# MrGreyPanda/NEM-MCMC-optimization

Hardware: AMD Instinct MI355X
Metric: order-score evals/sec (64 S-genes x 2000 effects); HBM GB/s fraction (higher is better)
Workload: dtype int8 fixed point 2^-38/ln2 + fp64 LSE

## Files before the change

nem-mcmc-optimization_amd/csrc/nemo_factored_i8.hip:

```cpp
#include "nemo_internal.h"

#include <math.h>

#include <string.h>

#include <algorithm>
#include <cmath>
#include <vector>

#ifndef NEMO_I8_ABLATE
#define NEMO_I8_ABLATE 0
#endif
#ifndef NEMO_I8L_RINIT
#define NEMO_I8L_RINIT 1
#endif
#ifndef NEMO_I8_WAVES_PER_SIMD
#define NEMO_I8_WAVES_PER_SIMD 2
#endif

namespace nemo {

namespace {

using i32x4 = __attribute__((ext_vector_type(4))) int;

constexpr double kPadG8 = -1.0e6;
constexpr int kARow = 6;
template <int ROWC>
__device__ __forceinline__ int a_byte(int i, int j) {
  if constexpr (ROWC == 4) return i * 64 + (((j >> 4) + 2 * ((i >> 2) & 3)) & 3) * 16 + (j & 15);
  else return i * (16 * ROWC) + j;
}

__device__ __forceinline__ double wsum(double v) {
#pragma unroll
  for (int o = 32; o >= 1; o >>= 1) v += __shfl_xor(v, o, kWave);
  return v;
// ... 129 lines not shown
  A8[1 * SL + off] = (int8_t)(((hb >> 12) & 63) - 32);
  A8[2 * SL + off] = (int8_t)(((hb >> 6) & 63) - 32);
  A8[3 * SL + off] = (int8_t)((hb & 63) - 32);
  A8[4 * SL + off] = (int8_t)(lb >> 18);
  A8[5 * SL + off] = (int8_t)(((lb >> 12) & 63) - 32);
  A8[6 * SL + off] = (int8_t)(((lb >> 6) & 63) - 32);
  A8[7 * SL + off] = (int8_t)((lb & 63) - 32);
}

constexpr double kL2Scale = 1512775.3951951857;

template <int SPAD, int ROWC>
__device__ __forceinline__ void i8l_digits(int8_t* A8, int i, int j, double d) {
  const double hd = rint(d * kL2Scale);
  const int h = (int)hd;
  const int l = (int)rint(fma(d, kL2Scale, -hd) * 262144.0);
  const int off = a_byte<ROWC>(i, j);
  const int hb = h + 32 * (1 + 64 + 4096), lb = l + 32 * (1 + 64);
  constexpr int SL = SPAD * 16 * ROWC;
  A8[0 * SL + off] = (int8_t)(hb >> 18);
  A8[1 * SL + off] = (int8_t)(((hb >> 12) & 63) - 32);
  A8[2 * SL + off] = (int8_t)(((hb >> 6) & 63) - 32);
  A8[3 * SL + off] = (int8_t)((hb & 63) - 32);
  A8[4 * SL + off] = (int8_t)(lb >> 12);
  A8[5 * SL + off] = (int8_t)(((lb >> 6) & 63) - 32);
  A8[6 * SL + off] = (int8_t)((lb & 63) - 32);
}

__device__ __forceinline__ double dswap32(double a, double b, double& out_b) {
  const uint64_t x = __builtin_bit_cast(uint64_t, a), y = __builtin_bit_cast(uint64_t, b);
  auto lo = __builtin_amdgcn_permlane32_swap((uint32_t)x, (uint32_t)y, false, false);
  auto hi = __builtin_amdgcn_permlane32_swap((uint32_t)(x >> 32), (uint32_t)(y >> 32), false, false);
  out_b = __builtin_bit_cast(double, ((uint64_t)hi[1] << 32) | lo[1]);
  return __builtin_bit_cast(double, ((uint64_t)hi[0] << 32) | lo[0]);
}
__device__ __forceinline__ double dswap16(double a, double b, double& out_b) {
  const uint64_t x = __builtin_bit_cast(uint64_t, a), y = __builtin_bit_cast(uint64_t, b);
  auto lo = __builtin_amdgcn_permlane16_swap((uint32_t)x, (uint32_t)y, false, false);
  auto hi = __builtin_amdgcn_permlane16_swap((uint32_t)(x >> 32), (uint32_t)(y >> 32), false, false);
  out_b = __builtin_bit_cast(double, ((uint64_t)hi[1] << 32) | lo[1]);
  return __builtin_bit_cast(double, ((uint64_t)hi[0] << 32) | lo[0]);
}

template <int SPAD, int WAVES, int KB, int ROWC, bool L2 = false>
__device__ __forceinline__ void i8o_prep_passes(EvalLds e, int k0, int w, int lane, int S, int cap,
                                                int cexp, const double* __restrict__ w01b,
                                                const double* __restrict__ elo_s,
// ... 324 lines not shown

constexpr double kL2C0 = 1.0000000000000377;
constexpr double kL2C1 = 2.521654728528023e-12;
constexpr double kL2C2 = 3.179908378901339e-24;

__device__ __forceinline__ uint64_t exp2_fx_load(uint32_t t0) {
#if NEMO_I8_ABLATE & 64
  const uint32_t addr = 0u;
#else
  const uint32_t addr = (t0 >> 6) & 0x3ff8u;
#endif
  return *(const __attribute__((address_space(3))) uint64_t*)(size_t)addr;
}
__device__ __forceinline__ double exp2_fx_series(uint32_t t0, int t1) {
  uint32_t rr;
  asm("v_lshl_add_u32 %0, %1, 18, %2" : "=v"(rr) : "v"(t0 & 511u), "v"((uint32_t)t1));
  const double r = (double)(int)rr;
  return fma(r, fma(r, kL2C2, kL2C1), kL2C0);
}
__device__ __forceinline__ double exp2_fx_series_r(int rr) {
  const double r = (double)rr;
  return fma(r, fma(r, kL2C2, kL2C1), kL2C0);
}
__device__ __forceinline__ double exp2_fx_apply(uint32_t t0, uint64_t ev, double p, double acc) {
  const uint32_t hi = (t0 & ~511u) ^ (uint32_t)(ev >> 32);
  return fma(__builtin_bit_cast(double, ((uint64_t)hi << 32) | (uint32_t)ev), p, acc);
}

template <int NR, int WAVES, bool DIAG>
__global__ __launch_bounds__(WAVES * kWave, NEMO_I8O_WAVES_PER_SIMD) void score_i8o_kernel(
    int S, int E, int ntiles, int nsets, int split, int cap, int cexp, double padg,
    const int32_t* __restrict__ pos, const double* __restrict__ w01,
    const double* __restrict__ e_lo, const double* __restrict__ e_hi,
    const uint8_t* __restrict__ B8, const double* __restrict__ Uoff,
    const int8_t* __restrict__ udig, const double* __restrict__ u0,
    const double* __restrict__ nullsum, const void* __restrict__ tabs, double sA, double sB,
    double* __restrict__ partial, double* __restrict__ ll_out, int remap) {
  constexpr int SPAD = NR * 16;
  constexpr int NP = 4;
  constexpr int NSL = 2 * NP;
  extern __shared__ __attribute__((aligned(16))) double lds8[];
  uint2* etab_o = (uint2*)lds8;
  double2* ltab = (double2*)(etab_o + kExpTabN);
  double* elo_s = (double*)(ltab + 128);
  double* ehi_s = elo_s + SPAD;
  EvalLds ev;
// ... 147 lines not shown
  }
}

template <int NR, int WAVES, bool DIAG>
hipError_t launch_i8o_t(Ctx& c, int batch, int cap, const int32_t* d_pos, const double* d_w01,
                        double* d_ll, hipStream_t st, int* nparts, bool* finalized) {
  constexpr int SPAD = NR * 16;
  const int ntiles = (c.E + 15) / 16;
  const int nsets = (ntiles + 7) / 8;
  const int slots = 256 * (NEMO_I8O_WAVES_PER_SIMD * 4 / WAVES);
  int split = (slots + batch - 1) / batch;
  split = split < 1 ? 1 : (split > nsets ? nsets : split);
  const size_t lds = kExpTabN * 8 + 128 * 16 + 3 * SPAD * 8 + 3 * SPAD * 4 + (size_t)8 * SPAD * 64;
  const double sA = ldexp(1.0, c.i8_cexp - 24), sB = ldexp(1.0, c.i8_cexp - 48);
  score_i8o_kernel<NR, WAVES, DIAG><<<dim3(batch * split), WAVES * kWave, lds, st>>>(
      c.S, c.E, ntiles, nsets, split, cap, c.i8_cexp, c.i8o_padg, d_pos, d_w01, c.d_elo, c.d_ehi,
      c.d_B8, c.d_Uoff, c.d_udig, c.d_u0, c.d_nullsum, c.d_i8o_tabs, sA, sB, fpartial(c), d_ll,
      c.xcd_remap);
  *nparts = nsets;
  *finalized = split == 1;
  return hipGetLastError();
}

template <int NR, int WAVES, class Hook>
__device__ __forceinline__ int i8l_walk2(const i32x4* __restrict__ Al0, const i32x4* __restrict__ Gi,
                                        const i32x4* __restrict__ Bt, const i32x4* __restrict__ Bt64,
                                        int set, int s_end, int ntiles, int E, int col, int lane,
                                        uint32_t a_lane, const double* __restrict__ nullsum,
                                        double* __restrict__ partial, size_t b, int nsets,
                                        const double2* __restrict__ ltab, Hook hook) {
  constexpr int SPAD = NR * 16;
  const int rg = lane >> 4;
  int it = 0;
  if (set < s_end) {
    double lprod = 1.0;
    int lexp = 0;
    int t = 8 * set;
    auto tend = [&](int st) { return min(ntiles, 8 * st + 8); };
    int t2 = t + 1 < tend(set) ? t + 1 : t;
    const __amdgpu_buffer_rsrc_t brs =
        __builtin_amdgcn_make_buffer_rsrc((void*)Bt, (short)0, 2 * ntiles * kWave * 16, 0x00020000);
    const uint32_t bln = (uint32_t)lane * 16u;
    auto bload = [&](int tile, int x64) {
      return __builtin_bit_cast(i32x4, __builtin_amdgcn_raw_buffer_load_b128(
                                           brs, bln, (x64 * ntiles + tile) * kWave * 16, 0));
    };
    i32x4 bca = bload(t, 0), bca64 = bload(t, 1);
    i32x4 bcb = bload(t2, 0), bcb64 = bload(t2, 1);
    for (;;) {
      uint32_t ao = a_lane;
      asm volatile("" : "+v"(ao));
      const i32x4* Al = Al0 + ao;
      const bool two = t2 != t;
      int tn = t + 2, setn = set;
      if (tn >= tend(set)) {
        setn = set + WAVES;
        tn = 8 * setn;
      }
      const bool more = setn < s_end;
      const int tla = __builtin_amdgcn_readfirstlane(more ? tn : t);
      const int tlb = __builtin_amdgcn_readfirstlane(more ? (tn + 1 < tend(setn) ? tn + 1 : tn) : t);
      const i32x4 b1a = bca, b64a = bca64, b1b = bcb, b64b = bcb64;
      bca = bload(tla, 0);
      bca64 = bload(tla, 1);
      bcb = bload(tlb, 0);
      bcb64 = bload(tlb, 1);
      double la0 = 0.0, la1 = 0.0, lb0 = 0.0, lb1 = 0.0;
#pragma unroll
      for (int r = 0; r < NR; ++r) {
        const i32x4 c0 = Gi[(16 * r) / 4 + rg];
        const i32x4 c1 = Gi[(SPAD + 16 * r) / 4 + rg];
        auto A = [&](int sl) { return Al[(sl * SPAD + 16 * r) * 4]; };
        i32x4 h0a, h0b, h1a, h1b, l0a, l0b, l1a, l1b;
        {
          const i32x4 a = A(0);
          h0a = __builtin_amdgcn_mfma_i32_16x16x64_i8(a, b64a, i32x4{0, 0, 0, 0}, 0, 0, 0);
          h0b = __builtin_amdgcn_mfma_i32_16x16x64_i8(a, b64b, i32x4{0, 0, 0, 0}, 0, 0, 0);
        }
        {
          const i32x4 a = A(1);
          h0a = __builtin_amdgcn_mfma_i32_16x16x64_i8(a, b1a, h0a, 0, 0, 0);
          h0b = __builtin_amdgcn_mfma_i32_16x16x64_i8(a, b1b, h0b, 0, 0, 0);
        }
        {
          const i32x4 a = A(2);
          h1a = __builtin_amdgcn_mfma_i32_16x16x64_i8(a, b64a, c0, 0, 0, 0);
          h1b = __builtin_amdgcn_mfma_i32_16x16x64_i8(a, b64b, c0, 0, 0, 0);
        }
        {
          const i32x4 a = A(3);
          h1a = __builtin_amdgcn_mfma_i32_16x16x64_i8(a, b1a, h1a, 0, 0, 0);
          h1b = __builtin_amdgcn_mfma_i32_16x16x64_i8(a, b1b, h1b, 0, 0, 0);
        }
#if NEMO_I8L_RINIT
        {
          const i32x4 a = A(5);
          l1a = __builtin_amdgcn_mfma_i32_16x16x64_i8(a, b64a, c1, 0, 0, 0);
          l1b = __builtin_amdgcn_mfma_i32_16x16x64_i8(a, b64b, c1, 0, 0, 0);
        }
        {
          const i32x4 a = A(6);
          l1a = __builtin_amdgcn_mfma_i32_16x16x64_i8(a, b1a, l1a, 0, 0, 0);
          l1b = __builtin_amdgcn_mfma_i32_16x16x64_i8(a, b1b, l1b, 0, 0, 0);
        }
        uint32_t t0a[4], t0b[4];
        uint64_t eva[4], evb[4];
        i32x4 ma, mb;
#pragma unroll
        for (int g = 0; g < 4; ++g) {
          t0a[g] = ((uint32_t)h0a[g] << 12) + (uint32_t)h1a[g];
          eva[g] = exp2_fx_load(t0a[g]);
          ma[g] = (int)((t0a[g] & 511u) << 6);
        }
#pragma unroll
        for (int g = 0; g < 4; ++g) {
          t0b[g] = ((uint32_t)h0b[g] << 12) + (uint32_t)h1b[g];
          evb[g] = exp2_fx_load(t0b[g]);
          mb[g] = (int)((t0b[g] & 511u) << 6);
        }
        {
          const i32x4 a = A(4);
          l0a = __builtin_amdgcn_mfma_i32_16x16x64_i8(a, b1a, ma, 0, 0, 0);
          l0b = __builtin_amdgcn_mfma_i32_16x16x64_i8(a, b1b, mb, 0, 0, 0);
        }
        auto epi = [&](const uint32_t (&t0)[4], const uint64_t (&evv)[4], const i32x4 l0, const i32x4 l1,
                       double& ls0, double& ls1) {
          double pr[4];
#pragma unroll
          for (int g = 0; g < 4; ++g) pr[g] = exp2_fx_series_r((int)(((uint32_t)l0[g] << 12) + (uint32_t)l1[g]));
#pragma unroll
          for (int g = 0; g < 4; ++g) {
            if (g & 1) ls1 = exp2_fx_apply(t0[g], evv[g], pr[g], ls1);
            else ls0 = exp2_fx_apply(t0[g], evv[g], pr[g], ls0);
          }
        };
        epi(t0a, eva, l0a, l1a, la0, la1);
        epi(t0b, evb, l0b, l1b, lb0, lb1);
#else
        {
          const i32x4 a = A(4);
          l0a = __builtin_amdgcn_mfma_i32_16x16x64_i8(a, b1a, i32x4{0, 0, 0, 0}, 0, 0, 0);
          l0b = __builtin_amdgcn_mfma_i32_16x16x64_i8(a, b1b, i32x4{0, 0, 0, 0}, 0, 0, 0);
        }
        {
          const i32x4 a = A(5);
          l1a = __builtin_amdgcn_mfma_i32_16x16x64_i8(a, b64a, c1, 0, 0, 0);
          l1b = __builtin_amdgcn_mfma_i32_16x16x64_i8(a, b64b, c1, 0, 0, 0);
        }
        {
          const i32x4 a = A(6);
          l1a = __builtin_amdgcn_mfma_i32_16x16x64_i8(a, b1a, l1a, 0, 0, 0);
          l1b = __builtin_amdgcn_mfma_i32_16x16x64_i8(a, b1b, l1b, 0, 0, 0);
        }
        auto epi = [&](const i32x4 h0, const i32x4 h1, const i32x4 l0, const i32x4 l1, double& ls0,
                       double& ls1) {
          uint32_t t0[4];
          uint64_t evv[4];
          double pr[4];
#pragma unroll
          for (int g = 0; g < 4; ++g) {
            t0[g] = ((uint32_t)h0[g] << 12) + (uint32_t)h1[g];
            evv[g] = exp2_fx_load(t0[g]);
          }
#pragma unroll
          for (int g = 0; g < 4; ++g)
            pr[g] = exp2_fx_series(t0[g], (int)(((uint32_t)l0[g] << 12) + (uint32_t)l1[g]));
#pragma unroll
          for (int g = 0; g < 4; ++g) {
            if (g & 1) ls1 = exp2_fx_apply(t0[g], evv[g], pr[g], ls1);
            else ls0 = exp2_fx_apply(t0[g], evv[g], pr[g], ls0);
          }
        };
        epi(h0a, h1a, l0a, l1a, la0, la1);
        epi(h0b, h1b, l0b, l1b, lb0, lb1);
#endif
      }
      const double l = rowsum_pair(la0 + la1, lb0 + lb1) + 1.0;
      const bool tb = (lane & 16) != 0;
      const bool ok = (((tb ? t2 : t) * 16 + col) < E) & (two | !tb);
      lprod *= ok ? l : 1.0;
      lexp += __builtin_amdgcn_frexp_exp(lprod);
      lprod = __builtin_amdgcn_frexp_mant(lprod);
      if (setn != set) {
        double v = log_fast(lprod, ltab) + (double)lexp * 0.69314718055994530942;
        v = rowsum16(v);
        v += __shfl_down(v, 16, kWave);
        if (lane == 0) partial[(size_t)b * nsets + set] = nullsum[set] + v;
        lprod = 1.0;
        lexp = 0;
      }
      hook(it++);
      if (!more) break;
      t = tn;
      t2 = tlb;
      set = setn;
    }
  }
  return it;
}

template <int NR, int WAVES, int OCC, int TT = 1, int MODE = 0>
__global__ __launch_bounds__(WAVES * kWave, OCC) void score_i8l_kernel(
    int S, int E, int ntiles, int nsets, int split, int cap, double padg,
    const int32_t* __restrict__ pos, const double* __restrict__ w01,
    const double* __restrict__ e_lo, const double* __restrict__ e_hi,
    const uint8_t* __restrict__ B8, const int8_t* __restrict__ udig, const double* __restrict__ u0,
    const double* __restrict__ nullsum, const void* __restrict__ tabs,
    double* __restrict__ partial, double* __restrict__ ll_out, int remap,
    int4* __restrict__ img = nullptr) {
  constexpr int SPAD = NR * 16;
  constexpr int NSL = 7;
  extern __shared__ __attribute__((aligned(16))) double lds8[];
  uint2* etab_o = (uint2*)lds8;
  double2* ltab = (double2*)(etab_o + kExpTabN);
  double* elo_s = (double*)(ltab + 128);
  double* ehi_s = elo_s + SPAD;
  EvalLds ev;
  ev.G = ehi_s + SPAD;
// ... 17 lines not shown
    const int4* src = (const int4*)tabs;
    int4* dst = (int4*)lds8;
    for (int k = tid + (MODE == 1 ? kExpTabN * 8 / 16 : 0); k < (kExpTabN * 8 + 128 * 16) / 16;
         k += blockDim.x)
      dst[k] = src[k];
    if constexpr (MODE != 2)
      for (int i = tid; i < SPAD; i += blockDim.x) {
        elo_s[i] = i < S ? e_lo[i] : 1.0;
        ehi_s[i] = i < S ? e_hi[i] : 1.0;
      }
  }
  if constexpr (MODE == 2) {
    const int4* src = img + (size_t)b * kImg4;
    int4* dst = (int4*)gi;
    for (int k = tid; k < kImg4; k += blockDim.x) dst[k] = src[k];
    __syncthreads();
  } else {
  i8_init_eval<SPAD, NSL, 4>(ev, pos + (size_t)b * S, S, tid, blockDim.x, padg);
  __syncthreads();
  {
    int8_t* A8 = (int8_t*)ev.A;
    for (int k = tid; k < S * NSL; k += blockDim.x) {
      const int i = k / NSL, sl = k - i * NSL;
      A8[sl * SPAD * 64 + a_byte<4>(i, i)] = udig[i * 8 + sl];
    }
  }
  {
    constexpr int KB = 4;
    const int npass = i8_npass(S, cap);
    const int my = npass > w ? (npass - w + WAVES - 1) / WAVES : 0;
    for (int k0 = 0; k0 < my; k0 += KB)
      i8o_prep_passes<SPAD, WAVES, KB, 4, true>(ev, k0, w, lane, S, cap, 0, w01 + (size_t)b * S * S,
                                                elo_s, ehi_s, ltab);
  }
  __syncthreads();
  for (int i = tid; i < SPAD; i += blockDim.x) {
    const double g = i < S ? ev.G[i] + u0[i] : ev.G[i];
    const double g0 = rint(g * kL2Scale);
    gi[i] = (int)g0 + (1023 << 20);
    gi[SPAD + i] = (int)rint(fma(g, kL2Scale, -g0) * 262144.0);
  }
  __syncthreads();
  if constexpr (MODE == 1) {
    const int4* src = (const int4*)gi;
    int4* dst = img + (size_t)b * kImg4;
    for (int k = tid; k < kImg4; k += blockDim.x) dst[k] = src[k];
    return;
// ... 42 lines not shown
  #endif
  #if NEMO_I8_ABLATE & 2
          const i32x4 h0 = A(0) + A(1) + b64, h1 = A(2) + A(3) + c0, l0 = A(4) + b1,
                      l1 = A(5) + A(6) + c1;
  #else
          i32x4 h0 = __builtin_amdgcn_mfma_i32_16x16x64_i8(A(0), b64, i32x4{0, 0, 0, 0}, 0, 0, 0);
          h0 = __builtin_amdgcn_mfma_i32_16x16x64_i8(A(1), b1, h0, 0, 0, 0);
          i32x4 h1 = __builtin_amdgcn_mfma_i32_16x16x64_i8(A(2), b64, c0, 0, 0, 0);
          h1 = __builtin_amdgcn_mfma_i32_16x16x64_i8(A(3), b1, h1, 0, 0, 0);
          const i32x4 l0 = __builtin_amdgcn_mfma_i32_16x16x64_i8(A(4), b1, i32x4{0, 0, 0, 0}, 0, 0, 0);
          i32x4 l1 = __builtin_amdgcn_mfma_i32_16x16x64_i8(A(5), b64, c1, 0, 0, 0);
          l1 = __builtin_amdgcn_mfma_i32_16x16x64_i8(A(6), b1, l1, 0, 0, 0);
  #endif
          uint32_t t0[4];
          uint64_t ev[4];
          double pr[4];
  #pragma unroll
          for (int g = 0; g < 4; ++g) {
            t0[g] = ((uint32_t)h0[g] << 12) + (uint32_t)h1[g];
            ev[g] = exp2_fx_load(t0[g]);
          }
  #pragma unroll
          for (int g = 0; g < 4; ++g)
            pr[g] = exp2_fx_series(t0[g], (int)(((uint32_t)l0[g] << 12) + (uint32_t)l1[g]));
  #pragma unroll
          for (int g = 0; g < 4; ++g) {
            if (g & 1) ls1 = exp2_fx_apply(t0[g], ev[g], pr[g], ls1);
            else ls0 = exp2_fx_apply(t0[g], ev[g], pr[g], ls0);
          }
        }
        double l = rowsum4(ls0 + ls1) + 1.0;
        lprod *= t * 16 + col < E ? l : 1.0;
        lexp += __builtin_amdgcn_frexp_exp(lprod);
        lprod = __builtin_amdgcn_frexp_mant(lprod);
        if (setn != set) {
          double v = log_fast(lprod, ltab) + (double)lexp * 0.69314718055994530942;
          v = rowsum16(v);
          if (lane == 0) partial[(size_t)b * nsets + set] = nullsum[set] + v;
          lprod = 1.0;
          lexp = 0;
        }
        if (!more) break;
        t = tn;
        set = setn;
      }
    }
  } else {
    i8l_walk2<NR, WAVES>(ev.A, Gi, Bt, Bt64, set, s_end, ntiles, E, col, lane, a_lane, nullsum, partial, b,
                         nsets, ltab, [](int) {});
  }
  if (split == 1) {
    __syncthreads();
    if (w == 0) {
      const double v = sum_partials(partial + (size_t)b * nsets, nsets, lane);
      if (lane == 0) ll_out[b] = v;
    }
  }
}

template <int NR>
__global__ __launch_bounds__(8 * kWave, NEMO_I8O_WAVES_PER_SIMD) void score_i8s_kernel(
    int S, int E, int ntiles, int nsets, int split, int cap, double padg,
    const int32_t* __restrict__ pos, const double* __restrict__ w01,
    const double* __restrict__ e_lo, const double* __restrict__ e_hi,
    const uint8_t* __restrict__ B8, const int8_t* __restrict__ udig, const double* __restrict__ u0,
    const double* __restrict__ nullsum, const void* __restrict__ tabs,
    double* __restrict__ partial, double* __restrict__ ll_out, int remap) {
  constexpr int WAVES = 8;
  constexpr int SPAD = NR * 16;
  constexpr int NSL = 7;
  constexpr int NG = WAVES / NR;
// ... 16 lines not shown
  const int s_begin = part * spb;
  const int s_end = min(nsets, s_begin + spb);
  const int tid = threadIdx.x;
  const int lane = tid & (kWave - 1);
  const int w = __builtin_amdgcn_readfirstlane(tid / kWave);
  const int rb = w % NR, grp = w / NR;
  const int col = lane & 15, rg = lane >> 4;

  {
    const int4* src = (const int4*)tabs;
    int4* dst = (int4*)lds8;
    for (int k = tid; k < (kExpTabN * 8 + 128 * 16) / 16; k += blockDim.x) dst[k] = src[k];
    for (int i = tid; i < SPAD; i += blockDim.x) {
      elo_s[i] = i < S ? e_lo[i] : 1.0;
      ehi_s[i] = i < S ? e_hi[i] : 1.0;
    }
  }
  i8_init_eval<SPAD, NSL, 4>(ev, pos + (size_t)b * S, S, tid, blockDim.x, padg);
  __syncthreads();
  {
    int8_t* A8 = (int8_t*)ev.A;
    for (int k = tid; k < S * NSL; k += blockDim.x) {
      const int i = k / NSL, sl = k - i * NSL;
      A8[sl * SPAD * 64 + a_byte<4>(i, i)] = udig[i * 8 + sl];
    }
  }
  {
    constexpr int KB = 4;
    const int npass = i8_npass(S, cap);
    const int my = npass > w ? (npass - w + WAVES - 1) / WAVES : 0;
    for (int k0 = 0; k0 < my; k0 += KB)
      i8o_prep_passes<SPAD, WAVES, KB, 4, true>(ev, k0, w, lane, S, cap, 0, w01 + (size_t)b * S * S,
                                                elo_s, ehi_s, ltab);
  }
  __syncthreads();
  for (int i = tid; i < SPAD; i += blockDim.x) {
    const double g = i < S ? ev.G[i] + u0[i] : ev.G[i];
    const double g0 = rint(g * kL2Scale);
    gi[i] = (int)g0 + (1023 << 20);
    gi[SPAD + i] = (int)rint(fma(g, kL2Scale, -g0) * 262144.0);
  }
  __syncthreads();
  i32x4 af[NSL];
  {
    const i32x4* Al = ev.A + (uint32_t)(col * 4 + ((rg + 2 * (col >> 2)) & 3));
#pragma unroll
    for (int sl = 0; sl < NSL; ++sl) af[sl] = Al[(sl * SPAD + 16 * rb) * 4];
// ... 17 lines not shown
      const int t_end = min(ntiles, 8 * set + 8);
      for (int t = 8 * set; t < t_end; ++t) {
        const int tn = t + 1 < t_end ? t + 1 : 8 * (set + NG);
        const i32x4 b1 = bc;
        const i32x4 b64 = b1 << 6;
        bc = Bt[(size_t)min(tn, ntiles - 1) * kWave + lane];
        const i32x4 h0 = __builtin_amdgcn_mfma_i32_16x16x64_i8(
            af[1], b1, __builtin_amdgcn_mfma_i32_16x16x64_i8(af[0], b64, i32x4{0, 0, 0, 0}, 0, 0, 0), 0, 0, 0);
        const i32x4 h1 = __builtin_amdgcn_mfma_i32_16x16x64_i8(
            af[3], b1, __builtin_amdgcn_mfma_i32_16x16x64_i8(af[2], b64, c0, 0, 0, 0), 0, 0, 0);
        const i32x4 l0 = __builtin_amdgcn_mfma_i32_16x16x64_i8(af[4], b1, i32x4{0, 0, 0, 0}, 0, 0, 0);
        const i32x4 l1 = __builtin_amdgcn_mfma_i32_16x16x64_i8(
            af[6], b1, __builtin_amdgcn_mfma_i32_16x16x64_i8(af[5], b64, c1, 0, 0, 0), 0, 0, 0);
        uint32_t t0[4];
        uint64_t evt[4];
        double pr[4];
#pragma unroll
        for (int g = 0; g < 4; ++g) {
          t0[g] = ((uint32_t)h0[g] << 12) + (uint32_t)h1[g];
          evt[g] = exp2_fx_load(t0[g]);
        }
#pragma unroll
        for (int g = 0; g < 4; ++g)
          pr[g] = exp2_fx_series(t0[g], (int)(((uint32_t)l0[g] << 12) + (uint32_t)l1[g]));
        double ls0 = 0.0, ls1 = 0.0;
#pragma unroll
        for (int g = 0; g < 4; ++g) {
          if (g & 1) ls1 = exp2_fx_apply(t0[g], evt[g], pr[g], ls1);
          else ls0 = exp2_fx_apply(t0[g], evt[g], pr[g], ls0);
        }
        const double v = rowsum4(ls0 + ls1);
        if (lane < 16) cs[((t - 8 * set) * NR + rb) * 16 + col] = v;
      }
    }
    __syncthreads();
    if (set < s_end && rb == k % NR) {
      double lp = 1.0;
      int le = 0;
#pragma unroll
      for (int h = 0; h < 2; ++h) {
        const int tt = (lane >> 4) + 4 * h;
        const int t = 8 * set + tt;
        double l = 1.0;
#pragma unroll
        for (int q = 0; q < NR; ++q) l += cs[(tt * NR + q) * 16 + col];
        lp *= t < ntiles && t * 16 + col < E ? l : 1.0;
        le += __builtin_amdgcn_frexp_exp(lp);
// ... 45 lines not shown
  const int lane = tid & (kWave - 1);
  const int w = __builtin_amdgcn_readfirstlane(tid / kWave);
  const int col = lane & 15, rg = lane >> 4;
  const int nb = gridDim.x;
  const int b0 = blockIdx.x;
  if (b0 >= batch) return;

  auto set_perm = [&](int k, int e) {
    int* perm = evb(k).perm;
    for (int j = tid; j < S; j += blockDim.x) {
      int pj = pos[(size_t)e * S + j];
      pj = pj < 0 ? 0 : (pj >= S ? S - 1 : pj);
      perm[pj] = j;
    }
  };
  auto zero_a = [&](int k) {
    i32x4* A = evb(k).A;
    for (int q = tid; q < NSL * SPAD * 4; q += blockDim.x) A[q] = i32x4{0, 0, 0, 0};
  };
  auto diag = [&](int k) {
    int8_t* A8 = (int8_t*)evb(k).A;
    for (int q = tid; q < S * NSL; q += blockDim.x) {
      const int i = q / NSL, sl = q - i * NSL;
      A8[sl * SPAD * 64 + a_byte<4>(i, i)] = udig[i * 8 + sl];
    }
  };
  auto prep = [&](int k, int e) {
    constexpr int KB = 4;
    const int npass = i8_npass(S, cap);
    const int my = npass > w ? (npass - w + WAVES - 1) / WAVES : 0;
    for (int k0 = 0; k0 < my; k0 += KB)
      i8o_prep_passes<SPAD, WAVES, KB, 4, true>(evb(k), k0, w, lane, S, cap, 0, w01 + (size_t)e * S * S,
                                                elo_s, ehi_s, ltab);
  };
  auto finalize_g = [&](int k) {
    const EvalLds ev = evb(k);
    int* gi = gib(k);
    for (int i = tid; i < SPAD; i += blockDim.x) {
      const double g = i < S ? ev.G[i] + u0[i] : ev.G[i];
      const double g0 = rint(g * kL2Scale);
      gi[i] = (int)g0 + (1023 << 20);
      gi[SPAD + i] = (int)rint(fma(g, kL2Scale, -g0) * 262144.0);
    }
  };

  {
    const int4* src = (const int4*)tabs;
// ... 6 lines not shown
  }
  for (int k = 0; k < 2; ++k) {
    for (int i = tid; i < SPAD; i += blockDim.x) evb(k).G[i] = i < S ? 0.0 : padg;
    zero_a(k);
  }
  set_perm(0, b0);
  if (b0 + nb < batch) set_perm(1, b0 + nb);
  __syncthreads();
  diag(0);
  diag(1);
  __syncthreads();
  prep(0, b0);
  __syncthreads();
  finalize_g(0);
  __syncthreads();

  const i32x4* Bt = (const i32x4*)B8;
  const i32x4* Bt64 = Bt + (size_t)ntiles * kWave;
  const uint32_t a_lane = (uint32_t)(col * 4 + ((rg + 2 * (col >> 2)) & 3));
  int k = 0;
  for (int e = b0; e < batch; e += nb, k ^= 1) {
    const int en = e + nb;
    bool pending = en < batch;
    i8l_walk2<NR, WAVES>(evb(k).A, (const i32x4*)gib(k), Bt, Bt64, w, nsets, ntiles, E, col, lane, a_lane,
                         nullsum, partial, (size_t)e, nsets, ltab, [&](int it) {
                           if (pending && it == 0) {
                             prep(k ^ 1, en);
                             pending = false;
                           }
                         });
    if (pending) prep(k ^ 1, en);
    __syncthreads();
    if (w == 0) {
      const double v = sum_partials(partial + (size_t)e * nsets, nsets, lane);
      if (lane == 0) ll_out[e] = v;
    }
    if (en < batch) finalize_g(k ^ 1);
    const bool again = en + nb < batch;
    if (again) {
      zero_a(k);
      set_perm(k, en + nb);
    }
    __syncthreads();
    if (again) diag(k);
  }
}

// ... 64 lines not shown
  } else {
    score_i8l_kernel<NR, WAVES, OCC, TT><<<dim3(batch * split), WAVES * kWave, lds, st>>>(
        c.S, c.E, ntiles, nsets, split, cap, c.i8o_padg, d_pos, d_w01, c.d_elo, c.d_ehi, c.d_B8,
        c.d_udig2, c.d_u0, c.d_nullsum, c.d_i8o_tabs, fpartial(c), d_ll, c.xcd_remap);
  }
  *nparts = nsets;
  *finalized = split == 1;
  return hipGetLastError();
}

constexpr int kWideKH = 2;

__device__ __forceinline__ void i8w_digits(int8_t* A8, int i, int j, double d) {
  constexpr int SPAD = 128, SL = SPAD * 64;
  const double hd = rint(d * kL2Scale);
  const int h = (int)hd;
  const int l = (int)rint(fma(d, kL2Scale, -hd) * 262144.0);
  const int off = (j >> 6) * SL + a_byte<4>(i, j & 63);
  const int hb = h + 32 * (1 + 64 + 4096), lb = l + 32 * (1 + 64);
  A8[(0 * kWideKH) * SL + off] = (int8_t)(hb >> 18);
  A8[(1 * kWideKH) * SL + off] = (int8_t)(((hb >> 12) & 63) - 32);
  A8[(2 * kWideKH) * SL + off] = (int8_t)(((hb >> 6) & 63) - 32);
  A8[(3 * kWideKH) * SL + off] = (int8_t)((hb & 63) - 32);
  A8[(4 * kWideKH) * SL + off] = (int8_t)(lb >> 12);
  A8[(5 * kWideKH) * SL + off] = (int8_t)(((lb >> 6) & 63) - 32);
  A8[(6 * kWideKH) * SL + off] = (int8_t)((lb & 63) - 32);
}

template <int WAVES, int KB>
__device__ __forceinline__ void i8w_prep_passes(EvalLds e, int k0, int w, int lane, int S, int cap,
                                                const double* __restrict__ w01b,
                                                const double* __restrict__ elo_s,
                                                const double* __restrict__ ehi_s,
                                                const double2* __restrict__ ltab) {
  const bool packed = cap == 0 || cap >= S - 1;
  const int npass = packed ? (S + 1) / 2 : S;
  int8_t* A8 = (int8_t*)e.A;
  double ga[KB], gb[KB];
#pragma unroll
  for (int kk = 0; kk < KB; ++kk) {
    ga[kk] = 0.0;
    gb[kk] = 0.0;
    const int q = w + (k0 + kk) * WAVES;
#pragma unroll
    for (int hr = 0; hr < kWideKH; ++hr) {
      const int p = lane + 64 * hr;
      int qr = 0, pp = 0;
// ... 57 lines not shown
  ev.A = (i32x4*)(ev.perm + SPAD);

  const int b = xcd_index8((int)blockIdx.x, (int)gridDim.x, remap);
  const int tid = threadIdx.x;
  const int lane = tid & (kWave - 1);
  const int w = __builtin_amdgcn_readfirstlane(tid / kWave);
  const int col = lane & 15, rg = lane >> 4;

  {
    const int4* src = (const int4*)tabs;
    int4* dst = (int4*)lds8;
    for (int k = tid; k < (kExpTabN * 8 + 128 * 16) / 16; k += blockDim.x) dst[k] = src[k];
    for (int i = tid; i < SPAD; i += blockDim.x) {
      elo_s[i] = i < S ? e_lo[i] : 1.0;
      ehi_s[i] = i < S ? e_hi[i] : 1.0;
    }
  }
  i8_init_eval<SPAD, NSL * kWideKH, 4>(ev, pos + (size_t)b * S, S, tid, blockDim.x, padg);
  __syncthreads();
  {
    int8_t* A8 = (int8_t*)ev.A;
    for (int k = tid; k < S * NSL; k += blockDim.x) {
      const int i = k / NSL, sl = k - i * NSL;
      A8[(sl * kWideKH + (i >> 6)) * SPAD * 64 + a_byte<4>(i, i & 63)] = udig[i * 8 + sl];
    }
  }
  {
    constexpr int KB = 2;
    const int npass = i8_npass(S, cap);
    const int my = npass > w ? (npass - w + WAVES - 1) / WAVES : 0;
    for (int k0 = 0; k0 < my; k0 += KB)
      i8w_prep_passes<WAVES, KB>(ev, k0, w, lane, S, cap, w01 + (size_t)b * S * S, elo_s, ehi_s, ltab);
  }
  __syncthreads();
  for (int i = tid; i < SPAD; i += blockDim.x) {
    const double g = i < S ? ev.G[i] + u0[i] : ev.G[i];
    const double g0 = rint(g * kL2Scale);
    gi[i] = (int)g0 + (1023 << 20);
    gi[SPAD + i] = (int)rint(fma(g, kL2Scale, -g0) * 262144.0);
  }
  __syncthreads();

  const i32x4* Gi = (const i32x4*)gi;
  const uint32_t a_lane = (uint32_t)(col * 4 + ((rg + 2 * (col >> 2)) & 3));
  const __amdgpu_buffer_rsrc_t brs =
      __builtin_amdgcn_make_buffer_rsrc((void*)B8, (short)0, 2 * kWideKH * ntiles * kWave * 16, 0x00020000);
  const uint32_t bln = (uint32_t)lane * 16u;
  auto bload = [&](int tile, int x64, int h) {
    return __builtin_bit_cast(i32x4, __builtin_amdgcn_raw_buffer_load_b128(
                                         brs, bln, ((x64 * kWideKH + h) * ntiles + tile) * kWave * 16, 0));
  };
  if constexpr (TWO) {
    for (int set = w; set < nsets; set += WAVES) {
      const int ta = kWideSetT * set;
      const bool two = ta + 1 < ntiles;
      const int tb = two ? ta + 1 : ta;
      const i32x4 b1a[2] = {bload(ta, 0, 0), bload(ta, 0, 1)}, b64a[2] = {bload(ta, 1, 0), bload(ta, 1, 1)};
      const i32x4 b1b[2] = {bload(tb, 0, 0), bload(tb, 0, 1)}, b64b[2] = {bload(tb, 1, 0), bload(tb, 1, 1)};
      uint32_t ao = a_lane;
      asm volatile("" : "+v"(ao));
      const i32x4* Al = ev.A + ao;
      double la0 = 0.0, la1 = 0.0, lb0 = 0.0, lb1 = 0.0;
#pragma unroll 1
      for (int r = 0; r < NR; ++r) {
        const i32x4 c0 = Gi[(16 * r) / 4 + rg];
        const i32x4 c1 = Gi[(SPAD + 16 * r) / 4 + rg];
        auto A = [&](int sl, int h) { return Al[((sl * kWideKH + h) * SPAD + 16 * r) * 4]; };
        i32x4 h0a = i32x4{0, 0, 0, 0}, h0b = i32x4{0, 0, 0, 0}, h1a = c0, h1b = c0;
        i32x4 l0a = i32x4{0, 0, 0, 0}, l0b = i32x4{0, 0, 0, 0}, l1a = c1, l1b = c1;
#pragma unroll
        for (int h = 0; h < kWideKH; ++h) {
          {
            const i32x4 a = A(0, h);
            h0a = __builtin_amdgcn_mfma_i32_16x16x64_i8(a, b64a[h], h0a, 0, 0, 0);
            h0b = __builtin_amdgcn_mfma_i32_16x16x64_i8(a, b64b[h], h0b, 0, 0, 0);
          }
          {
            const i32x4 a = A(1, h);
            h0a = __builtin_amdgcn_mfma_i32_16x16x64_i8(a, b1a[h], h0a, 0, 0, 0);
            h0b = __builtin_amdgcn_mfma_i32_16x16x64_i8(a, b1b[h], h0b, 0, 0, 0);
          }
          {
            const i32x4 a = A(2, h);
            h1a = __builtin_amdgcn_mfma_i32_16x16x64_i8(a, b64a[h], h1a, 0, 0, 0);
            h1b = __builtin_amdgcn_mfma_i32_16x16x64_i8(a, b64b[h], h1b, 0, 0, 0);
          }
          {
            const i32x4 a = A(3, h);
            h1a = __builtin_amdgcn_mfma_i32_16x16x64_i8(a, b1a[h], h1a, 0, 0, 0);
            h1b = __builtin_amdgcn_mfma_i32_16x16x64_i8(a, b1b[h], h1b, 0, 0, 0);
          }
          {
            const i32x4 a = A(4, h);
            l0a = __builtin_amdgcn_mfma_i32_16x16x64_i8(a, b1a[h], l0a, 0, 0, 0);
            l0b = __builtin_amdgcn_mfma_i32_16x16x64_i8(a, b1b[h], l0b, 0, 0, 0);
          }
          {
            const i32x4 a = A(5, h);
            l1a = __builtin_amdgcn_mfma_i32_16x16x64_i8(a, b64a[h], l1a, 0, 0, 0);
            l1b = __builtin_amdgcn_mfma_i32_16x16x64_i8(a, b64b[h], l1b, 0, 0, 0);
          }
          {
            const i32x4 a = A(6, h);
            l1a = __builtin_amdgcn_mfma_i32_16x16x64_i8(a, b1a[h], l1a, 0, 0, 0);
            l1b = __builtin_amdgcn_mfma_i32_16x16x64_i8(a, b1b[h], l1b, 0, 0, 0);
          }
        }
        auto epi = [&](const i32x4 h0, const i32x4 h1, const i32x4 l0, const i32x4 l1, double& ls0,
                       double& ls1) {
          uint32_t t0[4];
          uint64_t evv[4];
          double pr[4];
#pragma unroll
          for (int g = 0; g < 4; ++g) {
            t0[g] = ((uint32_t)h0[g] << 12) + (uint32_t)h1[g];
            evv[g] = exp2_fx_load(t0[g]);
          }
#pragma unroll
          for (int g = 0; g < 4; ++g)
            pr[g] = exp2_fx_series(t0[g], (int)(((uint32_t)l0[g] << 12) + (uint32_t)l1[g]));
#pragma unroll
          for (int g = 0; g < 4; ++g) {
            if (g & 1) ls1 = exp2_fx_apply(t0[g], evv[g], pr[g], ls1);
            else ls0 = exp2_fx_apply(t0[g], evv[g], pr[g], ls0);
          }
        };
        epi(h0a, h1a, l0a, l1a, la0, la1);
        epi(h0b, h1b, l0b, l1b, lb0, lb1);
      }
      const double l = rowsum_pair(la0 + la1, lb0 + lb1) + 1.0;
      const bool tile_b = (lane & 16) != 0;
      const bool ok = (((tile_b ? tb : ta) * 16 + col) < E) & (two | !tile_b);
      const double lprod = ok ? l : 1.0;
      double v = log_fast(lprod, ltab);
      v = rowsum16(v);
      v += __shfl_down(v, 16, kWave);
      if (lane == 0) partial[(size_t)b * nsets + set] = nullsum[set] + v;
    }
  } else {
    for (int set = w; set < nsets; set += WAVES) {
      double lprod = 1.0;
      int lexp = 0;
      const int t_end = min(ntiles, kWideSetT * set + kWideSetT);
      for (int t = kWideSetT * set; t < t_end; ++t) {
        const i32x4 b1[2] = {bload(t, 0, 0), bload(t, 0, 1)};
        const i32x4 b64[2] = {bload(t, 1, 0), bload(t, 1, 1)};
        uint32_t ao = a_lane;
        asm volatile("" : "+v"(ao));
        const i32x4* Al = ev.A + ao;
        double ls0 = 0.0, ls1 = 0.0;
  #pragma unroll 2
// ... 5 lines not shown
          h0 = __builtin_amdgcn_mfma_i32_16x16x64_i8(A(0, 1), b64[1], h0, 0, 0, 0);
          h0 = __builtin_amdgcn_mfma_i32_16x16x64_i8(A(1, 0), b1[0], h0, 0, 0, 0);
          h0 = __builtin_amdgcn_mfma_i32_16x16x64_i8(A(1, 1), b1[1], h0, 0, 0, 0);
          i32x4 h1 = __builtin_amdgcn_mfma_i32_16x16x64_i8(A(2, 0), b64[0], c0, 0, 0, 0);
          h1 = __builtin_amdgcn_mfma_i32_16x16x64_i8(A(2, 1), b64[1], h1, 0, 0, 0);
          h1 = __builtin_amdgcn_mfma_i32_16x16x64_i8(A(3, 0), b1[0], h1, 0, 0, 0);
          h1 = __builtin_amdgcn_mfma_i32_16x16x64_i8(A(3, 1), b1[1], h1, 0, 0, 0);
          i32x4 l0 = __builtin_amdgcn_mfma_i32_16x16x64_i8(A(4, 0), b1[0], i32x4{0, 0, 0, 0}, 0, 0, 0);
          l0 = __builtin_amdgcn_mfma_i32_16x16x64_i8(A(4, 1), b1[1], l0, 0, 0, 0);
          i32x4 l1 = __builtin_amdgcn_mfma_i32_16x16x64_i8(A(5, 0), b64[0], c1, 0, 0, 0);
          l1 = __builtin_amdgcn_mfma_i32_16x16x64_i8(A(5, 1), b64[1], l1, 0, 0, 0);
          l1 = __builtin_amdgcn_mfma_i32_16x16x64_i8(A(6, 0), b1[0], l1, 0, 0, 0);
          l1 = __builtin_amdgcn_mfma_i32_16x16x64_i8(A(6, 1), b1[1], l1, 0, 0, 0);
          uint32_t t0[4];
          uint64_t evv[4];
          double pr[4];
  #pragma unroll
          for (int g = 0; g < 4; ++g) {
            t0[g] = ((uint32_t)h0[g] << 12) + (uint32_t)h1[g];
            evv[g] = exp2_fx_load(t0[g]);
          }
  #pragma unroll
          for (int g = 0; g < 4; ++g)
            pr[g] = exp2_fx_series(t0[g], (int)(((uint32_t)l0[g] << 12) + (uint32_t)l1[g]));
  #pragma unroll
          for (int g = 0; g < 4; ++g) {
            if (g & 1) ls1 = exp2_fx_apply(t0[g], evv[g], pr[g], ls1);
            else ls0 = exp2_fx_apply(t0[g], evv[g], pr[g], ls0);
          }
        }
        const double l = rowsum4(ls0 + ls1) + 1.0;
        lprod *= t * 16 + col < E ? l : 1.0;
        lexp += __builtin_amdgcn_frexp_exp(lprod);
        lprod = __builtin_amdgcn_frexp_mant(lprod);
      }
      double v = log_fast(lprod, ltab) + (double)lexp * 0.69314718055994530942;
      v = rowsum16(v);
      if (lane == 0) partial[(size_t)b * nsets + set] = nullsum[set] + v;
    }
  }
  __syncthreads();
  if (w == 0) {
    const double v = sum_partials(partial + (size_t)b * nsets, nsets, lane);
    if (lane == 0) ll_out[b] = v;
  }
}

// ... 264 lines not shown
```

Baseline: 14.27 million.

## Fold low-residual init into MFMA accumulator and ping-pong B prefetch registers

Doubles the stored slice-4 digit and shifts the l0 partial by 11 instead of 12. The (t0 & 511) residual is now seeded into the l0 MFMA accumulator through a 16-bit shift, so the series no longer has to add it separately. The wide kernel now runs its l0 MFMAs after the table lookup and uses the cheaper series_r path. The walk loop is also turned into a lambda that is unrolled twice, swapping two B register sets instead of copying them each iteration. All of this reorders MFMA and epilogue work to cut VALU operations and register moves, at the cost of touching the fixed-point digit encoding, which risks numeric range issues.

```diff
diff --git a/nem-mcmc-optimization_amd/csrc/nemo_factored_i8.hip b/nem-mcmc-optimization_amd/csrc/nemo_factored_i8.hip
--- a/nem-mcmc-optimization_amd/csrc/nemo_factored_i8.hip
+++ b/nem-mcmc-optimization_amd/csrc/nemo_factored_i8.hip
@@ -13,6 +13,12 @@
 #endif
 #ifndef NEMO_I8L_RINIT
 #define NEMO_I8L_RINIT 1
+#endif
+#ifndef NEMO_I8L_CINIT16
+#define NEMO_I8L_CINIT16 1
+#endif
+#ifndef NEMO_I8L_PINGPONG
+#define NEMO_I8L_PINGPONG 1
 #endif
 #ifndef NEMO_I8_WAVES_PER_SIMD
 #define NEMO_I8_WAVES_PER_SIMD 2
@@ -188,7 +194,7 @@
   A8[1 * SL + off] = (int8_t)(((hb >> 12) & 63) - 32);
   A8[2 * SL + off] = (int8_t)(((hb >> 6) & 63) - 32);
   A8[3 * SL + off] = (int8_t)((hb & 63) - 32);
-  A8[4 * SL + off] = (int8_t)(lb >> 12);
+  A8[4 * SL + off] = (int8_t)(2 * (lb >> 12));
   A8[5 * SL + off] = (int8_t)(((lb >> 6) & 63) - 32);
   A8[6 * SL + off] = (int8_t)((lb & 63) - 32);
 }
@@ -559,6 +565,15 @@
   const double r = (double)rr;
   return fma(r, fma(r, kL2C2, kL2C1), kL2C0);
 }
+__device__ __forceinline__ int i8l_cinit16(uint32_t t0) {
+#if NEMO_I8L_CINIT16
+  int r;
+  asm("v_lshlrev_b16 %0, 7, %1" : "=v"(r) : "v"(t0));
+  return r;
+#else
+  return (int)((t0 & 511u) << 7);
+#endif
+}
 __device__ __forceinline__ double exp2_fx_apply(uint32_t t0, uint64_t ev, double p, double acc) {
   const uint32_t hi = (t0 & ~511u) ^ (uint32_t)(ev >> 32);
   return fma(__builtin_bit_cast(double, ((uint64_t)hi << 32) | (uint32_t)ev), p, acc);
@@ -752,7 +767,7 @@
   return hipGetLastError();
 }
 
-template <int NR, int WAVES, class Hook>
+template <int NR, int WAVES, bool PP, class Hook>
 __device__ __forceinline__ int i8l_walk2(const i32x4* __restrict__ Al0, const i32x4* __restrict__ Gi,
                                         const i32x4* __restrict__ Bt, const i32x4* __restrict__ Bt64,
                                         int set, int s_end, int ntiles, int E, int col, int lane,
@@ -777,7 +792,8 @@
     };
     i32x4 bca = bload(t, 0), bca64 = bload(t, 1);
     i32x4 bcb = bload(t2, 0), bcb64 = bload(t2, 1);
-    for (;;) {
+    auto iter = [&](const i32x4 b1a, const i32x4 b64a, const i32x4 b1b, const i32x4 b64b, i32x4& na,
+                    i32x4& na64, i32x4& nb, i32x4& nb64) -> bool {
       uint32_t ao = a_lane;
       asm volatile("" : "+v"(ao));
       const i32x4* Al = Al0 + ao;
@@ -790,11 +806,10 @@
       const bool more = setn < s_end;
       const int tla = __builtin_amdgcn_readfirstlane(more ? tn : t);
       const int tlb = __builtin_amdgcn_readfirstlane(more ? (tn + 1 < tend(setn) ? tn + 1 : tn) : t);
-      const i32x4 b1a = bca, b64a = bca64, b1b = bcb, b64b = bcb64;
-      bca = bload(tla, 0);
-      bca64 = bload(tla, 1);
-      bcb = bload(tlb, 0);
-      bcb64 = bload(tlb, 1);
+      na = bload(tla, 0);
+      na64 = bload(tla, 1);
+      nb = bload(tlb, 0);
+      nb64 = bload(tlb, 1);
       double la0 = 0.0, la1 = 0.0, lb0 = 0.0, lb1 = 0.0;
 #pragma unroll
       for (int r = 0; r < NR; ++r) {
@@ -840,13 +855,13 @@
         for (int g = 0; g < 4; ++g) {
           t0a[g] = ((uint32_t)h0a[g] << 12) + (uint32_t)h1a[g];
           eva[g] = exp2_fx_load(t0a[g]);
-          ma[g] = (int)((t0a[g] & 511u) << 6);
+          ma[g] = i8l_cinit16(t0a[g]);
         }
 #pragma unroll
         for (int g = 0; g < 4; ++g) {
           t0b[g] = ((uint32_t)h0b[g] << 12) + (uint32_t)h1b[g];
           evb[g] = exp2_fx_load(t0b[g]);
-          mb[g] = (int)((t0b[g] & 511u) << 6);
+          mb[g] = i8l_cinit16(t0b[g]);
         }
         {
           const i32x4 a = A(4);
@@ -857,7 +872,7 @@
                        double& ls0, double& ls1) {
           double pr[4];
 #pragma unroll
-          for (int g = 0; g < 4; ++g) pr[g] = exp2_fx_series_r((int)(((uint32_t)l0[g] << 12) + (uint32_t)l1[g]));
+          for (int g = 0; g < 4; ++g) pr[g] = exp2_fx_series_r((int)(((uint32_t)l0[g] << 11) + (uint32_t)l1[g]));
 #pragma unroll
           for (int g = 0; g < 4; ++g) {
             if (g & 1) ls1 = exp2_fx_apply(t0[g], evv[g], pr[g], ls1);
@@ -894,7 +909,7 @@
           }
 #pragma unroll
           for (int g = 0; g < 4; ++g)
-            pr[g] = exp2_fx_series(t0[g], (int)(((uint32_t)l0[g] << 12) + (uint32_t)l1[g]));
+            pr[g] = exp2_fx_series(t0[g], (int)(((uint32_t)l0[g] << 11) + (uint32_t)l1[g]));
 #pragma unroll
           for (int g = 0; g < 4; ++g) {
             if (g & 1) ls1 = exp2_fx_apply(t0[g], evv[g], pr[g], ls1);
@@ -920,10 +935,28 @@
         lexp = 0;
       }
       hook(it++);
-      if (!more) break;
+      if (!more) return false;
       t = tn;
       t2 = tlb;
       set = setn;
+      return true;
+    };
+    if constexpr (PP) {
+      i32x4 bqa, bqa64, bqb, bqb64;
+      for (;;) {
+        if (!iter(bca, bca64, bcb, bcb64, bqa, bqa64, bqb, bqb64)) break;
+        if (!iter(bqa, bqa64, bqb, bqb64, bca, bca64, bcb, bcb64)) break;
+      }
+    } else {
+      for (;;) {
+        i32x4 na, na64, nb, nb64;
+        const bool more = iter(bca, bca64, bcb, bcb64, na, na64, nb, nb64);
+        bca = na;
+        bca64 = na64;
+        bcb = nb;
+        bcb64 = nb64;
+        if (!more) break;
+      }
     }
   }
   return it;
@@ -987,7 +1020,8 @@
     int8_t* A8 = (int8_t*)ev.A;
     for (int k = tid; k < S * NSL; k += blockDim.x) {
       const int i = k / NSL, sl = k - i * NSL;
-      A8[sl * SPAD * 64 + a_byte<4>(i, i)] = udig[i * 8 + sl];
+      const int8_t d = udig[i * 8 + sl];
+      A8[sl * SPAD * 64 + a_byte<4>(i, i)] = sl == 4 ? (int8_t)(2 * d) : d;
     }
   }
   {
@@ -1076,7 +1110,7 @@
           }
   #pragma unroll
           for (int g = 0; g < 4; ++g)
-            pr[g] = exp2_fx_series(t0[g], (int)(((uint32_t)l0[g] << 12) + (uint32_t)l1[g]));
+            pr[g] = exp2_fx_series(t0[g], (int)(((uint32_t)l0[g] << 11) + (uint32_t)l1[g]));
   #pragma unroll
           for (int g = 0; g < 4; ++g) {
             if (g & 1) ls1 = exp2_fx_apply(t0[g], ev[g], pr[g], ls1);
@@ -1100,7 +1134,7 @@
       }
     }
   } else {
-    i8l_walk2<NR, WAVES>(ev.A, Gi, Bt, Bt64, set, s_end, ntiles, E, col, lane, a_lane, nullsum, partial, b,
+    i8l_walk2<NR, WAVES, NEMO_I8L_PINGPONG != 0>(ev.A, Gi, Bt, Bt64, set, s_end, ntiles, E, col, lane, a_lane, nullsum, partial, b,
                          nsets, ltab, [](int) {});
   }
   if (split == 1) {
@@ -1163,7 +1197,8 @@
     int8_t* A8 = (int8_t*)ev.A;
     for (int k = tid; k < S * NSL; k += blockDim.x) {
       const int i = k / NSL, sl = k - i * NSL;
-      A8[sl * SPAD * 64 + a_byte<4>(i, i)] = udig[i * 8 + sl];
+      const int8_t d = udig[i * 8 + sl];
+      A8[sl * SPAD * 64 + a_byte<4>(i, i)] = sl == 4 ? (int8_t)(2 * d) : d;
     }
   }
   {
@@ -1227,7 +1262,7 @@
         }
 #pragma unroll
         for (int g = 0; g < 4; ++g)
-          pr[g] = exp2_fx_series(t0[g], (int)(((uint32_t)l0[g] << 12) + (uint32_t)l1[g]));
+          pr[g] = exp2_fx_series(t0[g], (int)(((uint32_t)l0[g] << 11) + (uint32_t)l1[g]));
         double ls0 = 0.0, ls1 = 0.0;
 #pragma unroll
         for (int g = 0; g < 4; ++g) {
@@ -1319,7 +1354,8 @@
     int8_t* A8 = (int8_t*)evb(k).A;
     for (int q = tid; q < S * NSL; q += blockDim.x) {
       const int i = q / NSL, sl = q - i * NSL;
-      A8[sl * SPAD * 64 + a_byte<4>(i, i)] = udig[i * 8 + sl];
+      const int8_t d = udig[i * 8 + sl];
+      A8[sl * SPAD * 64 + a_byte<4>(i, i)] = sl == 4 ? (int8_t)(2 * d) : d;
     }
   };
   auto prep = [&](int k, int e) {
@@ -1372,7 +1408,7 @@
   for (int e = b0; e < batch; e += nb, k ^= 1) {
     const int en = e + nb;
     bool pending = en < batch;
-    i8l_walk2<NR, WAVES>(evb(k).A, (const i32x4*)gib(k), Bt, Bt64, w, nsets, ntiles, E, col, lane, a_lane,
+    i8l_walk2<NR, WAVES, false>(evb(k).A, (const i32x4*)gib(k), Bt, Bt64, w, nsets, ntiles, E, col, lane, a_lane,
                          nullsum, partial, (size_t)e, nsets, ltab, [&](int it) {
                            if (pending && it == 0) {
                              prep(k ^ 1, en);
@@ -1483,7 +1519,7 @@
   A8[(1 * kWideKH) * SL + off] = (int8_t)(((hb >> 12) & 63) - 32);
   A8[(2 * kWideKH) * SL + off] = (int8_t)(((hb >> 6) & 63) - 32);
   A8[(3 * kWideKH) * SL + off] = (int8_t)((hb & 63) - 32);
-  A8[(4 * kWideKH) * SL + off] = (int8_t)(lb >> 12);
+  A8[(4 * kWideKH) * SL + off] = (int8_t)(2 * (lb >> 12));
   A8[(5 * kWideKH) * SL + off] = (int8_t)(((lb >> 6) & 63) - 32);
   A8[(6 * kWideKH) * SL + off] = (int8_t)((lb & 63) - 32);
 }
@@ -1587,7 +1623,8 @@
     int8_t* A8 = (int8_t*)ev.A;
     for (int k = tid; k < S * NSL; k += blockDim.x) {
       const int i = k / NSL, sl = k - i * NSL;
-      A8[(sl * kWideKH + (i >> 6)) * SPAD * 64 + a_byte<4>(i, i & 63)] = udig[i * 8 + sl];
+      const int8_t d = udig[i * 8 + sl];
+      A8[(sl * kWideKH + (i >> 6)) * SPAD * 64 + a_byte<4>(i, i & 63)] = sl == 4 ? (int8_t)(2 * d) : d;
     }
   }
   {
@@ -1632,7 +1669,7 @@
         const i32x4 c1 = Gi[(SPAD + 16 * r) / 4 + rg];
         auto A = [&](int sl, int h) { return Al[((sl * kWideKH + h) * SPAD + 16 * r) * 4]; };
         i32x4 h0a = i32x4{0, 0, 0, 0}, h0b = i32x4{0, 0, 0, 0}, h1a = c0, h1b = c0;
-        i32x4 l0a = i32x4{0, 0, 0, 0}, l0b = i32x4{0, 0, 0, 0}, l1a = c1, l1b = c1;
+        i32x4 l1a = c1, l1b = c1;
 #pragma unroll
         for (int h = 0; h < kWideKH; ++h) {
           {
@@ -1656,11 +1693,6 @@
             h1b = __builtin_amdgcn_mfma_i32_16x16x64_i8(a, b1b[h], h1b, 0, 0, 0);
           }
           {
-            const i32x4 a = A(4, h);
-            l0a = __builtin_amdgcn_mfma_i32_16x16x64_i8(a, b1a[h], l0a, 0, 0, 0);
-            l0b = __builtin_amdgcn_mfma_i32_16x16x64_i8(a, b1b[h], l0b, 0, 0, 0);
-          }
-          {
             const i32x4 a = A(5, h);
             l1a = __builtin_amdgcn_mfma_i32_16x16x64_i8(a, b64a[h], l1a, 0, 0, 0);
             l1b = __builtin_amdgcn_mfma_i32_16x16x64_i8(a, b64b[h], l1b, 0, 0, 0);
@@ -1671,27 +1703,40 @@
             l1b = __builtin_amdgcn_mfma_i32_16x16x64_i8(a, b1b[h], l1b, 0, 0, 0);
           }
         }
-        auto epi = [&](const i32x4 h0, const i32x4 h1, const i32x4 l0, const i32x4 l1, double& ls0,
-                       double& ls1) {
-          uint32_t t0[4];
-          uint64_t evv[4];
+        uint32_t t0a[4], t0b[4];
+        uint64_t eva[4], evb[4];
+        i32x4 l0a, l0b;
+#pragma unroll
+        for (int g = 0; g < 4; ++g) {
+          t0a[g] = ((uint32_t)h0a[g] << 12) + (uint32_t)h1a[g];
+          eva[g] = exp2_fx_load(t0a[g]);
+          l0a[g] = i8l_cinit16(t0a[g]);
+        }
+#pragma unroll
+        for (int g = 0; g < 4; ++g) {
+          t0b[g] = ((uint32_t)h0b[g] << 12) + (uint32_t)h1b[g];
+          evb[g] = exp2_fx_load(t0b[g]);
+          l0b[g] = i8l_cinit16(t0b[g]);
+        }
+#pragma unroll
+        for (int h = 0; h < kWideKH; ++h) {
+          const i32x4 a = A(4, h);
+          l0a = __builtin_amdgcn_mfma_i32_16x16x64_i8(a, b1a[h], l0a, 0, 0, 0);
+          l0b = __builtin_amdgcn_mfma_i32_16x16x64_i8(a, b1b[h], l0b, 0, 0, 0);
+        }
+        auto epi = [&](const uint32_t (&t0)[4], const uint64_t (&evv)[4], const i32x4 l0, const i32x4 l1,
+                       double& ls0, double& ls1) {
           double pr[4];
 #pragma unroll
-          for (int g = 0; g < 4; ++g) {
-            t0[g] = ((uint32_t)h0[g] << 12) + (uint32_t)h1[g];
-            evv[g] = exp2_fx_load(t0[g]);
-          }
-#pragma unroll
-          for (int g = 0; g < 4; ++g)
-            pr[g] = exp2_fx_series(t0[g], (int)(((uint32_t)l0[g] << 12) + (uint32_t)l1[g]));
+          for (int g = 0; g < 4; ++g) pr[g] = exp2_fx_series_r((int)(((uint32_t)l0[g] << 11) + (uint32_t)l1[g]));
 #pragma unroll
           for (int g = 0; g < 4; ++g) {
             if (g & 1) ls1 = exp2_fx_apply(t0[g], evv[g], pr[g], ls1);
             else ls0 = exp2_fx_apply(t0[g], evv[g], pr[g], ls0);
           }
         };
-        epi(h0a, h1a, l0a, l1a, la0, la1);
-        epi(h0b, h1b, l0b, l1b, lb0, lb1);
+        epi(t0a, eva, l0a, l1a, la0, la1);
+        epi(t0b, evb, l0b, l1b, lb0, lb1);
       }
       const double l = rowsum_pair(la0 + la1, lb0 + lb1) + 1.0;
       const bool tile_b = (lane & 16) != 0;
@@ -1743,7 +1788,7 @@
           }
   #pragma unroll
           for (int g = 0; g < 4; ++g)
-            pr[g] = exp2_fx_series(t0[g], (int)(((uint32_t)l0[g] << 12) + (uint32_t)l1[g]));
+            pr[g] = exp2_fx_series(t0[g], (int)(((uint32_t)l0[g] << 11) + (uint32_t)l1[g]));
   #pragma unroll
           for (int g = 0; g < 4; ++g) {
             if (g & 1) ls1 = exp2_fx_apply(t0[g], evv[g], pr[g], ls1);
```

Result: faster. 14.71 million (median of 6 runs) (+3.1%).
